# rfrazier716/PyRayT

Hardware: AMD Instinct MI355X
Metric: ray-surface intersections/sec, 1M-ray biconvex lens (higher is better)
Workload: dtype f64

## Files before the change

include/prt.h:

```cpp
#ifndef PRT_H
#define PRT_H

#include <stdint.h>

#ifdef __cplusplus
extern "C" {
#endif

#define PRT_VERSION 240

enum {
  PRT_ROW_OX = 0, PRT_ROW_OY = 1, PRT_ROW_OZ = 2, PRT_ROW_OW = 3,
  PRT_ROW_DX = 4, PRT_ROW_DY = 5, PRT_ROW_DZ = 6, PRT_ROW_DW = 7,
  PRT_ROW_GENERATION = 8, PRT_ROW_INTENSITY = 9, PRT_ROW_WAVELENGTH = 10,
  PRT_ROW_INDEX = 11, PRT_ROW_ID = 12,
  PRT_RAY_ROWS = 13
};

enum {
  PRT_COL_GENERATION = 0, PRT_COL_INTENSITY = 1, PRT_COL_WAVELENGTH = 2, PRT_COL_INDEX = 3,
  PRT_COL_ID = 4, PRT_COL_SURFACE = 5, PRT_COL_X0 = 6, PRT_COL_Y0 = 7, PRT_COL_Z0 = 8,
  PRT_COL_X1 = 9, PRT_COL_Y1 = 10, PRT_COL_Z1 = 11, PRT_COL_XTILT = 12, PRT_COL_YTILT = 13,
  PRT_COL_ZTILT = 14,
  PRT_RECORD_COLS = 15
// ... 52 lines not shown

typedef struct prt_scene_options {
  int32_t struct_size;
  int32_t no_chain;
  int32_t no_cull;
  int32_t cull_min;
  int32_t no_groups;
  int32_t no_implied;
  int32_t hit_lanes;
  int32_t hit_staged;
  int32_t list_order_groups;
  int32_t one_direction;
  int32_t no_intervals;
  int32_t no_clearance;
  int32_t no_plane_bound;
  int32_t reserved[3];
} prt_scene_options;

int prt_scene_create(const prt_prim* prims, int n_prims, const prt_node* nodes, int n_nodes,
                     const int32_t* roots, int n_roots, const prt_material* mats, int n_mats,
                     const prt_scene_options* options, prt_scene** out);
void prt_scene_destroy(prt_scene* scene);
int prt_scene_update(prt_scene* scene, const prt_prim* prims, int n_prims, const prt_node* nodes, int n_nodes,
                     const int32_t* roots, int n_roots, const prt_material* mats, int n_mats,
                     const prt_scene_options* options);
int prt_scene_set_index_tables(prt_scene* scene, const int64_t* ranges, int n_mats, const double* wavelengths,
                               const double* indices, int64_t total);
int prt_scene_component_rows(const prt_scene* scene, int root);
int prt_scene_info(const prt_scene* scene, int64_t* out10);


// ... 216 lines not shown
                                                     int64_t max_group_rows);
int prt_frame_design_sensitivity(int device, const double* rows, int64_t ld, const int64_t* rows_per_generation,
                                 int n_generations, double id0, int64_t n_ids, const prt_prim* surfaces, int n_surfaces,
                                 const double* twists, const int64_t* parameter_ids, const int32_t* parameter_first,
                                 const double* linear, const double* index_rates, const int64_t* index_ids,
                                 const int32_t* index_first, int n_parameters, const int64_t* row_slot,
                                 const int64_t* selected, int64_t n_selected, const int64_t* group_first, int n_groups,
                                 int weight_column, const double* pivots, double* jacobian_out, double* sums_out,
                                 int64_t* record_out, void* workspace, void* stream);

#define PRT_VARIANT_FUSED 1
#define PRT_VARIANT_UNFUSED 2
#define PRT_VARIANT_KLANES 3
int prt_trace_stats(const prt_scene* scene, double* out8);
int prt_trace_telemetry(const prt_scene* scene, int64_t* out12);
int prt_trace_shortcut_counts(const prt_scene* scene, int64_t* out1);

typedef struct prt_camera {
  double world[16];
  int64_t h_pixels, v_pixels;
  double h_width, v_width;
} prt_camera;

int prt_camera_rays(int device, const prt_camera* camera, int64_t first, int64_t count,
                    double* rays_out, int64_t ld, void* stream);

int prt_render_hits(prt_scene* scene, int device, const double* rays, int64_t n, int64_t ld,
                    double* t_out, int64_t* surf_out, void* stream);

int prt_gooch_shade(prt_scene* scene, int device, const double* rays, int64_t n, int64_t ld,
                    const double* t, const int64_t* surf, const double* gooch,
// ... 53 lines not shown
```

pyrayt_amd/csrc/prt_abi_states.hpp:

```cpp
#pragma once
extern "C" int prt_version(void) { return PRT_VERSION; }
extern "C" const char* prt_last_error(void) { return g_error.c_str(); }
extern "C" int prt_device_count(void) {
  int count = 0;
  if (hipGetDeviceCount(&count) != hipSuccess) return 0;
  return count;
}

static inline unsigned blocks_for(int64_t n) { return (unsigned)((n + PRT_BLOCK - 1) / PRT_BLOCK); }
static inline size_t lds_bytes(int slots) { return (size_t)slots * PRT_BLOCK * 12; }
static inline size_t align_up(size_t v, size_t a) { return (v + a - 1) / a * a; }
static inline size_t lds_bytes_fused(int slots) {
  return (size_t)((3 * slots + 1) / 2 + 8) * PRT_BLOCK * sizeof(double);
}

static SceneDev trace_scene_dev(const prt_scene* s, const DeviceCopy* c) {
  SceneDev sd{c->prims, c->trace_code, (int)s->trace_program.code.size(), s->trace_program.lds_slots};
  for (size_t p = 0; p < s->dev_prims.size() && p < 64; ++p)
    if (s->dev_prims[p].mat_kind == MAT_ABSORBER) sd.absorber_mask |= 1ull << p;
  return sd;
}

struct HitVariant {
  int lanes = 1;
// ... 190 lines not shown
  const InteractLayout l = interact_layout(n);
  char* w = (char*)workspace;
  TraceCtrl* ctrl = (TraceCtrl*)(w + l.ctrl);
  int32_t* counts = (int32_t*)(w + l.counts);
  int64_t* offsets = (int64_t*)(w + l.offsets);
  hipLaunchKernelGGL(k_ctrl_init, dim3(1), dim3(1), 0, st, ctrl, n, ld_rows);
  if (n > 0) {
    SceneDev sd{c->prims, nullptr, (int)s->prims.size(), 0};
    hipLaunchKernelGGL(k_count, dim3(blocks_for(n)), dim3(PRT_BLOCK), 0, st, sd,
                       (int)s->prims.size(), rays_in, ld_in, n, surf, counts);
    hipLaunchKernelGGL(k_scan, dim3(1), dim3(1024), 0, st, counts, offsets, ctrl);
    const int relaunch = (generation + 1 != generation_limit) ? 1 : 0;
    hipLaunchKernelGGL(k_shade, dim3(blocks_for(n)), dim3(PRT_BLOCK), 0, st, sd, rays_in, ld_in,
                       (const TraceCtrl*)ctrl, n, t, (const int32_t*)nullptr, surf,
                       (const int64_t*)offsets, rays_out, ld_out, rows_out, ld_rows, (int64_t)0,
                       (double)(generation + 1), relaunch, ray_offset, 1, ctrl, shaded, ld_shaded);
  }
  hipLaunchKernelGGL(k_interact_finish, dim3(1), dim3(1), 0, st, (const TraceCtrl*)ctrl, n_live_out);
  HIP_TRY(hipGetLastError());
  return PRT_OK;
}

#include "prt_host_shade.hpp"
```

pyrayt_amd/csrc/prt_device.hpp:

```cpp
#pragma once
#include <hip/hip_runtime.h>
#include <stdint.h>

#include "prt_math.hpp"

#ifndef PRT_BLOCK
#define PRT_BLOCK 256
#endif
#define PRT_INF (__builtin_inf())

struct DevPrim {
  double minv[16];
  double params[6];
  double coef[6];
  double surface_id;
  int32_t type, mat_kind, normal_scale, pad;
};

typedef const __attribute__((address_space(4))) DevPrim* ConstPrimPtr;
__device__ __forceinline__ ConstPrimPtr const_prim(const DevPrim* prims, int index) {
  return (ConstPrimPtr)(unsigned long long)(prims + index);
}

enum { I_LEAF = 0, I_CSG = 1, I_ROOT = 2, I_BOX = 3, I_CHAIN = 4 };
enum { BOX_TEST = 0, BOX_PICK = 1, BOX_JUMP = 2, BOX_LINE = 3 };
enum { OPER_REGA = 0, OPER_REGB = 1, OPER_LDS = 2 };
enum { CSG_UNION = 1, CSG_INTERSECT = 2, CSG_DIFFERENCE = 3 };
enum { PRIM_SPHERE = 0, PRIM_CYLINDER = 1, PRIM_PLANE = 2, PRIM_CUBE = 3, PRIM_PARABOLOID = 4 };
enum { MAT_NONE = 0, MAT_ABSORBER = 1, MAT_MIRROR = 2, MAT_CONST = 3, MAT_SELLMEIER = 4, MAT_TABLE = 5, MAT_HOST = 6 };

struct DevInstr {
// ... 16 lines not shown
  int32_t shape;
  int32_t n_leaves;
  int32_t op1, op2;
  int32_t prim[3];
  int32_t implied1, implied2;
  int32_t clearance;
  int32_t intervals;
  double box1[6], box2[6];
  double leaf[3][18];
};
static_assert(sizeof(DevChain) == 3 * sizeof(DevInstr), "a chain record spans three step slots");
enum { CHAIN_SLOTS = 3 };
enum {
  CHAIN_SSC = 0, CHAIN_SSQ, CHAIN_CSS, CHAIN_QSS, CHAIN_QQQ,
  CHAIN_SC, CHAIN_SQ, CHAIN_CS, CHAIN_QS, CHAIN_CB, CHAIN_QB, CHAIN_PC, CHAIN_PQ, CHAIN_BC,
  CHAIN_SHAPES
};

struct Ray8 {
  double ox, oy, oz, ow, dx, dy, dz, dw;
  bool gated;
  bool any_w;
  bool lex;
  unsigned long long* paths;
};

#define kWellFormedLen2Lo 0.81
__device__ __forceinline__ bool well_formed(const Ray8& r) {
  if (!r.gated) return false;
  const double len2 = (r.dx * r.dx + r.dy * r.dy) + r.dz * r.dz;
// ... 204 lines not shown
  t0 = fmin(h0, h1);
  t1 = fmax(h0, h1);
}
__device__ __forceinline__ void surface_pair(int type, const double* __restrict__ q,
                                             const double* __restrict__ m, const Ray8& r,
                                             double& t0, double& t1) {
  const double ox = row_dot(m, 0, r.ox, r.oy, r.oz, r.ow);
  const double oy = row_dot(m, 1, r.ox, r.oy, r.oz, r.ow);
  const double oz = row_dot(m, 2, r.ox, r.oy, r.oz, r.ow);
  const double dx = row_dot(m, 0, r.dx, r.dy, r.dz, r.dw);
  const double dy = row_dot(m, 1, r.dx, r.dy, r.dz, r.dw);
  const double dz = row_dot(m, 2, r.dx, r.dy, r.dz, r.dw);
  object_pair(type, q, ox, oy, oz, dx, dy, dz, t0, t1);
}

__device__ __forceinline__ void plane_leaf_candidate(const double* __restrict__ q, const double* __restrict__ m,
                                                     const Ray8& r, int p, double& best_t, int& best_prim) {
  const double oz = row_dot(m, 2, r.ox, r.oy, r.oz, r.ow);
  const double dz = row_dot(m, 2, r.dx, r.dy, r.dz, r.dw);
  const bool skew = near0(dz);
  double t = -oz / (dz + (skew ? 1.0 : 0.0));
  if (skew) t = PRT_INF;
  const bool can = t > 0 && t < PRT_INF && beats(r, t, p, best_t, best_prim);
  if (__ballot(can) == 0ull) {
    count_wave(r.paths, 4);
    return;
  }
  const double ox = row_dot(m, 0, r.ox, r.oy, r.oz, r.ow);
  const double oy = row_dot(m, 1, r.ox, r.oy, r.oz, r.ow);
  const double dx = row_dot(m, 0, r.dx, r.dy, r.dz, r.dw);
// ... 26 lines not shown
    case PRIM_PLANE:
      ax = 0.0; ay = 0.0; az = 1.0;
      normalise = false;
      break;
    case PRIM_CUBE:
      ax = close_to(lx, q[1]) ? 1.0 : (close_to(lx, q[0]) ? -1.0 : 0.0);
      ay = close_to(ly, q[3]) ? 1.0 : (close_to(ly, q[2]) ? -1.0 : 0.0);
      az = close_to(lz, q[5]) ? 1.0 : (close_to(lz, q[4]) ? -1.0 : 0.0);
      break;
    default:
      ax = lx; ay = ly; az = -2 * q[0];
      if (close_to(lz, q[1])) { ax = 0.0; ay = 0.0; az = 1.0; }
      break;
  }
  if (normalise) {
    const double len = norm4(ax, ay, az, 0.0);
    div3(ax, ay, az, len, ax, ay, az);
  }
}

template <class PrimPtr>
__device__ __forceinline__ void world_normal_len(PrimPtr p, double px, double py, double pz, double pw,
                                                 double& nx, double& ny, double& nz, double& len_out) {
  const auto m = p->minv;
  const double lx = row_dot(m, 0, px, py, pz, pw);
  const double ly = row_dot(m, 1, px, py, pz, pw);
  const double lz = row_dot(m, 2, px, py, pz, pw);
  const auto q = p->params;
  double ax, ay, az;
  bool normalise = true;
  switch (p->type) {
// ... 8 lines not shown
    case PRIM_PLANE:
      ax = 0.0; ay = 0.0; az = 1.0;
      normalise = false;
      break;
    case PRIM_CUBE:
      ax = close_to(lx, q[1]) ? 1.0 : (close_to(lx, q[0]) ? -1.0 : 0.0);
      ay = close_to(ly, q[3]) ? 1.0 : (close_to(ly, q[2]) ? -1.0 : 0.0);
      az = close_to(lz, q[5]) ? 1.0 : (close_to(lz, q[4]) ? -1.0 : 0.0);
      break;
    default:
      ax = lx; ay = ly; az = -2 * q[0];
      if (close_to(lz, q[1])) { ax = 0.0; ay = 0.0; az = 1.0; }
      break;
  }
  if (normalise) {
    const double len = norm4(ax, ay, az, 0.0);
    ax /= len; ay /= len; az /= len;
  }
  double wx = col_dot(m, 0, ax, ay, az, 0.0);
  double wy = col_dot(m, 1, ax, ay, az, 0.0);
  double wz = col_dot(m, 2, ax, ay, az, 0.0);
  const double len = norm4(wx, wy, wz, 0.0);
  const double sgn = (double)p->normal_scale;
  div3(wx, wy, wz, len, wx, wy, wz);
  nx = wx * sgn;
  ny = wy * sgn;
  nz = wz * sgn;
  len_out = len;
}
template <class PrimPtr>
__device__ __forceinline__ void world_normal(PrimPtr p, double px, double py, double pz, double pw,
                                             double& nx, double& ny, double& nz) {
  double len;
  world_normal_len(p, px, py, pz, pw, nx, ny, nz, len);
}

template <class PrimPtr>
// ... 23 lines not shown
                  (k[2] * w2) / (w2 - k[5]));
}

__device__ __forceinline__ void reflect4(double& dx, double& dy, double& dz, double& dw, double nx,
                                         double ny, double nz, double nw) {
  const double dot = ((dx * nx + dy * ny) + dz * nz) + dw * nw;
  dx = dx - (2 * nx) * dot;
  dy = dy - (2 * ny) * dot;
  dz = dz - (2 * nz) * dot;
  dw = dw - (2 * nw) * dot;
}

__device__ __forceinline__ void refract4(double vx, double vy, double vz, double vw, double nx,
                                         double ny, double nz, double nw, double n1, double n2_in,
                                         double n_global, double& ox, double& oy, double& oz,
                                         double& ow, double& index_out) {
  const double cos_p = ((vx * nx + vy * ny) + vz * nz) + vw * nw;
  const double cos_n = ((vx * -nx + vy * -ny) + vz * -nz) + vw * -nw;
  const bool leaving = cos_p > 0;
  const double n2 = leaving ? n_global : n2_in;
  const double mx = leaving ? -nx : nx, my = leaving ? -ny : ny, mz = leaving ? -nz : nz,
               mw = leaving ? -nw : nw;
  const double r = n1 / n2;
  const double cos1 = leaving ? cos_p : cos_n;
  const double radicand = 1 - (r * r) * (1 - cos1 * cos1);
  const double cos2 = prt_sqrt_clamped(radicand);
  double ux, uy, uz, uw;
  if (radicand > 0) {
    const double k = r * cos1 - cos2;
    ux = r * vx + k * mx; uy = r * vy + k * my; uz = r * vz + k * mz; uw = r * vw + k * mw;
  } else {
    const double k = 2 * cos1;
    ux = vx + k * mx; uy = vy + k * my; uz = vz + k * mz; uw = vw + k * mw;
  }
  const double ulen = norm4(ux, uy, uz, uw);
  div3(ux, uy, uz, ulen, ox, oy, oz);
  ow = uw;
  if (uw != 0.0 || !(ulen > 0.0 && ulen < PRT_INF)) ow = uw / ulen;
  index_out = (radicand > 0) ? n2 : n1;
}

template <class PrimPtr>
__device__ __forceinline__ int shade(PrimPtr p, double px, double py, double pz, double pw, double& dx,
                                     double& dy, double& dz, double& dw, double wavelength,
                                     double& index, double tx, double ty, double tz) {
  const int kind = p->mat_kind;
  if (kind == MAT_NONE || kind == MAT_HOST) return -5;
  if (kind == MAT_ABSORBER) {
    dx = 0.0; dy = 0.0; dz = 0.0; dw = 0.0;
    return 0;
  }
  double nx, ny, nz;
  world_normal(p, px, py, pz, pw, nx, ny, nz);
  const double nw = 0.0 * (double)p->normal_scale;
  if (kind == MAT_MIRROR) {
    reflect4(dx, dy, dz, dw, nx, ny, nz, nw);
    return 0;
  }
  bool found;
  const double n_mat = glass_index(p, wavelength, found);
  double vx = tx, vy = ty, vz = tz, vw = dw;
  if (dw != 0.0) {
    const double len = norm4(dx, dy, dz, dw);
    vx = dx / len; vy = dy / len; vz = dz / len; vw = dw / len;
  }
  refract4(vx, vy, vz, vw, nx, ny, nz, nw, index, n_mat, 1.0, dx, dy, dz, dw, index);
  return found ? 0 : -6;
}

extern __shared__ double lds_dyn[];

struct LaneLists {
  int total;
  int off;
  __device__ __forceinline__ double get_t(int slot) const {
    return lds_dyn[(off + slot) * PRT_BLOCK + threadIdx.x];
  }
  __device__ __forceinline__ int get_id(int slot) const {
    return reinterpret_cast<const int*>(lds_dyn + total * PRT_BLOCK)[(off + slot) * PRT_BLOCK + threadIdx.x];
  }
  __device__ __forceinline__ void put(int slot, double v, int i) const {
// ... 311 lines not shown
  return inside;
}

__device__ __forceinline__ void offer_chord(const Ray8& ray, bool some, double lo, double hi, int id_lo, int id_hi,
                                            double& best_t, int& best_prim) {
  const bool first = some && lo > 0;
  const bool second = some && hi > 0 && hi < PRT_INF;
  const double t = first ? lo : (second ? hi : PRT_INF);
  const int prim = first ? id_lo : (second ? id_hi : -1);
  if (beats(ray, t, prim, best_t, best_prim)) {
    best_t = t;
    best_prim = prim;
  }
}

template <int T0, int T1, int T2>
__device__ __forceinline__ void chain_candidate(const DevChain* __restrict__ ch, const Ray8& ray,
                                                double& best_t, int& best_prim) {
  double lv[2], rv[2], r2[2] = {PRT_INF, PRT_INF};
  const int id0 = ch->prim[0], id1 = ch->prim[1];
  bool have_third = false;
  if (T0 == PRIM_CYLINDER && T2 >= 0 && ch->intervals != 0 && ch->clearance != 0) {
    surface_pair(T1, ch->leaf[1], ch->leaf[1] + 6, ray, rv[0], rv[1]);
    surface_pair(T2 < 0 ? 0 : T2, ch->leaf[2], ch->leaf[2] + 6, ray, r2[0], r2[1]);
    have_third = true;
    const int id2 = ch->prim[2];
    const bool b_in = r2[0] >= rv[0], b_out = r2[1] < rv[1];
    const double lo = b_in ? r2[0] : rv[0], hi = b_out ? r2[1] : rv[1];
    const bool tie = lo == hi && hi < PRT_INF;
    bool some = lo < hi;
    const bool wanted = (some && hi > 0) || tie;
    if (__ballot(wanted) == 0ull) return;
    if (__ballot(wanted && (tie || !chord_inside_cylinder(ch->leaf[0], ch->leaf[0] + 6, ray, lo, hi))) == 0ull) {
      some = some && implied_touch(ch->box1, ray, some, lo, hi);
      some = some && implied_touch(ch->box2, ray, some, lo, hi);
      offer_chord(ray, some, lo, hi, b_in ? id2 : id1, b_out ? id2 : id1, best_t, best_prim);
      return;
    }
    surface_pair(T0, ch->leaf[0], ch->leaf[0] + 6, ray, lv[0], lv[1]);
  } else {
    surface_pair(T0, ch->leaf[0], ch->leaf[0] + 6, ray, lv[0], lv[1]);
    surface_pair(T1, ch->leaf[1], ch->leaf[1] + 6, ray, rv[0], rv[1]);
  }
  if (ch->intervals != 0) {
    const bool b_in = rv[0] >= lv[0], b_out = rv[1] < lv[1];
    double lo = b_in ? rv[0] : lv[0], hi = b_out ? rv[1] : lv[1];
    int id_lo = b_in ? id1 : id0, id_hi = b_out ? id1 : id0;
    bool undecided = lo == hi && hi < PRT_INF;
    bool some = lo < hi;
    some = some && implied_touch(ch->box1, ray, some, lo, hi);
    if (T2 >= 0) {
      const bool wanted = (some && hi > 0) || undecided;
      if (__ballot(wanted) == 0ull) return;
      bool cut = true;
// ... 44 lines not shown
    csg_keep<4, 2>(op2, l4, r2, ch->box2, ray, implied2, keep4, keep2, c2);
    const int id2 = ch->prim[2];
    const int lid[4] = {id0, id0, id1, id1}, rid[2] = {id2, id2};
    csg_root_pick<4, 2>(l4, lid, keep4, r2, rid, keep2, t, prim);
  }
  if (beats(ray, t, prim, best_t, best_prim)) {
    best_t = t;
    best_prim = prim;
  }
}

__device__ __forceinline__ void chain_step(const DevChain* __restrict__ ch, int shape, const Ray8& ray,
                                           double& best_t, int& best_prim) {
  switch (shape) {
    case CHAIN_SSC: chain_candidate<PRIM_SPHERE, PRIM_SPHERE, PRIM_CYLINDER>(ch, ray, best_t, best_prim); break;
    case CHAIN_SSQ: chain_candidate<PRIM_SPHERE, PRIM_SPHERE, PRIM_CUBE>(ch, ray, best_t, best_prim); break;
    case CHAIN_CSS: chain_candidate<PRIM_CYLINDER, PRIM_SPHERE, PRIM_SPHERE>(ch, ray, best_t, best_prim); break;
    case CHAIN_QSS: chain_candidate<PRIM_CUBE, PRIM_SPHERE, PRIM_SPHERE>(ch, ray, best_t, best_prim); break;
    case CHAIN_QQQ: chain_candidate<PRIM_CUBE, PRIM_CUBE, PRIM_CUBE>(ch, ray, best_t, best_prim); break;
    case CHAIN_SC: chain_candidate<PRIM_SPHERE, PRIM_CYLINDER, -1>(ch, ray, best_t, best_prim); break;
    case CHAIN_SQ: chain_candidate<PRIM_SPHERE, PRIM_CUBE, -1>(ch, ray, best_t, best_prim); break;
    case CHAIN_CS: chain_candidate<PRIM_CYLINDER, PRIM_SPHERE, -1>(ch, ray, best_t, best_prim); break;
    case CHAIN_QS: chain_candidate<PRIM_CUBE, PRIM_SPHERE, -1>(ch, ray, best_t, best_prim); break;
    case CHAIN_CB: chain_candidate<PRIM_CYLINDER, PRIM_PARABOLOID, -1>(ch, ray, best_t, best_prim); break;
    case CHAIN_QB: chain_candidate<PRIM_CUBE, PRIM_PARABOLOID, -1>(ch, ray, best_t, best_prim); break;
    case CHAIN_PC: chain_candidate<PRIM_PLANE, PRIM_CYLINDER, -1>(ch, ray, best_t, best_prim); break;
    case CHAIN_PQ: chain_candidate<PRIM_PLANE, PRIM_CUBE, -1>(ch, ray, best_t, best_prim); break;
    default: chain_candidate<PRIM_PARABOLOID, PRIM_CYLINDER, -1>(ch, ray, best_t, best_prim); break;
  }
}
// ... 175 lines not shown
```

pyrayt_amd/csrc/prt_scene.hpp:

```cpp
#pragma once
static thread_local std::string g_error;

static int fail(int code, const std::string& msg) {
  g_error = msg;
  return code;
}

#define HIP_TRY(expr)                                                                        \
  do {                                                                                       \
    hipError_t e_ = (expr);                                                                  \
    if (e_ != hipSuccess)                                                                    \
      return fail(PRT_ERR_HIP, std::string(#expr) + ": " + hipGetErrorString(e_));          \
  } while (0)

static const int kMaxBatch = 64;
struct SceneDev {
  const DevPrim* prims;
  const DevInstr* code;
  int n_instr;
  int lds_slots;
  unsigned long long absorber_mask = 0;
};

struct Program {
// ... 92 lines not shown
  std::vector<int64_t> table_ranges;
  std::vector<double> table_wavelengths, table_indices;
  bool has_cull_steps = false;
  bool spatial_groups = false;
  int stats_device = -1, stats_ticket = 0;
  int last_generations = 0;
  long lookback_fallbacks = 0;
  int64_t hint_n = -1;
  int hint_keep_absorbed = 0;
  std::vector<char> hint_mode;
  long speculation_misses = 0;
  bool full_rows = false;
  long full_rows_fallbacks = 0;
  long dense_launches = 0;
  long sparse_keep_launches = 0;
  long long path_counts[5] = {0, 0, 0, 0, 0};
  int hint_holdoff = 0;
  std::vector<char> missed_mode;
  std::vector<int> hint_rest, hint_rest_span;
  int hint_misses_in_a_row = 0;
};

static int leaves_under(const prt_scene* s, int node) {
  const prt_node& n = s->nodes[node];
  if (n.op == PRT_NODE_LEAF) return 1;
  return leaves_under(s, n.left) + leaves_under(s, n.right);
}

static bool solid_bounds(const prt_scene* s, int node, double* box);

static double short_direction_bound(const prt_scene* s, int node);
// ... 261 lines not shown
  out->implied1 = c.box_contains_solid(nodes[0]) ? 1 : 0;
  for (int k = 0; k < 6; ++k) out->box1[k] = s->nodes[nodes[0]].aabb[k];
  if (n_leaves == 3) {
    out->op2 = s->nodes[nodes[1]].op;
    out->implied2 = c.box_contains_solid(nodes[1]) ? 1 : 0;
    for (int k = 0; k < 6; ++k) out->box2[k] = s->nodes[nodes[1]].aabb[k];
  }
  for (int k = 0; k < n_leaves; ++k) {
    const int prim = s->nodes[leaves[k]].prim;
    const prt_prim& pr = s->prims[prim];
    out->prim[k] = prim;
    for (int j = 0; j < 6; ++j) out->leaf[k][j] = pr.params[j];
    for (int j = 0; j < 12; ++j) out->leaf[k][6 + j] = pr.minv[j];
  }
  out->clearance = s->options.no_clearance ? 0 : 1;
  out->intervals = (out->op1 == PRT_NODE_INTERSECT && out->implied1 && (n_leaves == 2 || (out->op2 == PRT_NODE_INTERSECT && out->implied2))) ? 1 : 0;
  if (s->options.no_intervals) out->intervals = 0;
  return true;
}
static Operand compile_component(const prt_scene* s, int root_node, std::vector<DevInstr>& code,
                                 int root_rule, int* slots) {
  size_t box_at = (size_t)-1;
  const bool cull_off = s->options.no_cull != 0;
  const int cull_min = s->options.cull_min > 0 ? s->options.cull_min : 3;
  const bool line_cull = root_rule == ROOT_RENDER && !cull_off;
  if ((root_rule == ROOT_TRACE && (int)s->roots.size() >= cull_min && !cull_off) || line_cull) {
    DevInstr in = Compiler::blank(I_BOX);
    in.a1 = line_cull ? BOX_LINE : BOX_TEST;
    double* box = in.data;
    if (solid_bounds(s, root_node, box) && short_direction_bound(s, root_node) <= kWellFormedLen2Lo) {
// ... 365 lines not shown
    }
    const prt_material& m = s->mats[p.material];
    if (m.kind < PRT_MAT_NONE || m.kind > PRT_MAT_HOST) {
      delete s;
      return fail(PRT_ERR_SCENE, "unknown material kind");
    }
    DevPrim d;
    std::memset(&d, 0, sizeof(d));
    std::memcpy(d.minv, p.minv, sizeof(d.minv));
    std::memcpy(d.params, p.params, sizeof(d.params));
    std::memcpy(d.coef, m.coef, sizeof(d.coef));
    d.surface_id = (double)p.surface_id;
    d.type = p.type;
    d.mat_kind = m.kind;
    d.normal_scale = p.normal_scale < 0 ? -1 : 1;
    if (m.kind == PRT_MAT_NONE || m.kind == PRT_MAT_HOST || m.kind == PRT_MAT_TABLE) s->has_untracable = true;
    if (m.kind == PRT_MAT_TABLE) {
      const double nan_index = m.coef[3];
      std::memset(d.coef, 0, sizeof(d.coef));
      d.coef[3] = nan_index;
    }
    s->dev_prims.push_back(d);
  }
  compile_trace_program(s);
  if (const char* wrong = verify_program(s, s->trace_program, true)) {
    const std::string message = std::string("internal error, the compiled trace program is malformed: ") + wrong;
    delete s;
    return fail(PRT_ERR_SCENE, message);
  }
  s->has_cull_steps = count_steps(s->trace_program.code, I_BOX) > 0;
// ... 313 lines not shown
```

pyrayt_amd/csrc/prt_trace_kernels.hpp:

```cpp
#pragma once
__device__ __forceinline__ LaneLists lane_lists(int slots) { return LaneLists{slots, 0}; }

__device__ __forceinline__ Ray8 load_ray8(const double* __restrict__ rays, int64_t ld, int64_t i) {
  Ray8 r;
  r.ox = rays[0 * ld + i]; r.oy = rays[1 * ld + i]; r.oz = rays[2 * ld + i]; r.ow = rays[3 * ld + i];
  r.dx = rays[4 * ld + i]; r.dy = rays[5 * ld + i]; r.dz = rays[6 * ld + i]; r.dw = rays[7 * ld + i];
  r.gated = false;
  r.any_w = true;
  r.lex = false;
  r.paths = nullptr;
  return r;
}

struct TraceCtrl {
  int64_t n_cur;
  int64_t n_live;
  int64_t n_carry;
  int64_t row_base;
  int64_t rows_cap;
  int32_t error;
  int32_t pad;
  unsigned long long paths[6];
};

// ... 185 lines not shown

struct Meta5 {
  double generation, intensity, wavelength, index, id;
};
__device__ __forceinline__ Meta5 load_meta(const double* __restrict__ rays, int64_t ld, int64_t i) {
  Meta5 m;
  m.generation = rays[8 * ld + i];
  m.intensity = rays[9 * ld + i];
  m.wavelength = rays[10 * ld + i];
  m.index = rays[11 * ld + i];
  m.id = rays[12 * ld + i];
  return m;
}

__device__ __forceinline__ Shaded interact_compute(const SceneDev& scene, const Meta5& m, const Ray8& r,
                                                   double t, int prim) {
  Shaded s;
  s.generation = m.generation;
  s.intensity = m.intensity;
  s.wavelength = m.wavelength;
  s.index_in = m.index;
  s.id = m.id;
  s.px = r.ox + r.dx * t; s.py = r.oy + r.dy * t; s.pz = r.oz + r.dz * t; s.pw = r.ow + r.dw * t;
  s.dx = r.dx; s.dy = r.dy; s.dz = r.dz; s.dw = r.dw;
  s.index = s.index_in;
  s.surface_id = -1.0;
  s.err = 0;
  const double tilt = norm3(r.dx, r.dy, r.dz);
  div3(r.dx, r.dy, r.dz, tilt, s.tx, s.ty, s.tz);
  unsigned long long todo = __ballot(true);
  while (todo) {
    const int leader = __ffsll((long long)todo) - 1;
    const int cur = __shfl(prim, leader);
    if (prim == cur) {
      const DevPrim* __restrict__ p = scene.prims + cur;
      s.err = shade(p, s.px, s.py, s.pz, s.pw, s.dx, s.dy, s.dz, s.dw, s.wavelength, s.index,
                   s.tx, s.ty, s.tz);
      s.surface_id = p->surface_id;
    }
    todo &= ~__ballot(prim == cur);
  }
  return s;
}

__device__ __forceinline__ void interact_store(const Shaded& s, const Ray8& r, bool carry, int64_t row,
                                               int64_t j, double* __restrict__ next, int64_t ld_next,
                                               double* __restrict__ rows, int64_t ld_rows,
                                               double next_generation, int relaunch, double ray_offset) {
  rows[PRT_COL_GENERATION * ld_rows + row] = s.generation;
  rows[PRT_COL_INTENSITY * ld_rows + row] = s.intensity;
  rows[PRT_COL_WAVELENGTH * ld_rows + row] = s.wavelength;
  rows[PRT_COL_INDEX * ld_rows + row] = s.index_in;
// ... 35 lines not shown
                                              bool carry, int64_t row, int64_t j,
                                              double* __restrict__ next, int64_t ld_next,
                                              double* __restrict__ rows, int64_t ld_rows,
                                              double next_generation, int relaunch, double ray_offset) {
  const Shaded s = interact_compute(scene, load_meta(rays, ld, i), r, t, prim);
  interact_store(s, r, carry, row, j, next, ld_next, rows, ld_rows, next_generation, relaunch, ray_offset);
  return s.err;
}

__global__ void __launch_bounds__(PRT_BLOCK)
k_shade(SceneDev scene, const double* __restrict__ rays, int64_t ld, const TraceCtrl* __restrict__ ctrl_in,
        int64_t n_fixed, const double* __restrict__ hit_t, const int32_t* __restrict__ hit_prim,
        const int64_t* __restrict__ hit_surf, const int64_t* __restrict__ block_offsets,
        double* __restrict__ next, int64_t ld_next, double* __restrict__ rows, int64_t ld_rows,
        int64_t row_base_fixed, double next_generation, int relaunch, double ray_offset,
        int keep_absorbed, TraceCtrl* __restrict__ ctrl, const double* __restrict__ shaded, int64_t ld_shaded) {
  __shared__ int s_wave[4];
  const int64_t n = ctrl_in ? ctrl_in->n_cur : n_fixed;
  if (ctrl_in && (ctrl_in->error != 0 || ctrl_in->n_live == 0)) return;
  const int64_t row_base = ctrl_in ? ctrl_in->row_base : row_base_fixed;
  const int64_t i = (int64_t)blockIdx.x * PRT_BLOCK + threadIdx.x;
  const bool in_range = i < n;
  Ray8 r = {0, 0, 0, 1, 0, 0, 0, 0};
  double t = PRT_INF;
  int prim = -1;
  if (in_range) {
    r = load_ray8(rays, ld, i);
    t = hit_t[i];
    if (hit_prim) {
      prim = hit_prim[i];
    } else {
      prim = prim_of_surface(scene.prims, scene.n_instr, hit_surf[i]);
    }
  }
  const bool live = in_range && is_live(r, prim);
  const bool carry = live && (keep_absorbed || scene.prims[prim].mat_kind != MAT_ABSORBER);
  const int live_rank = block_rank(live, s_wave);
  const int carry_rank = block_rank(carry, s_wave);
  if (!live) return;

  const int64_t row = row_base + block_offsets[2 * blockIdx.x] + live_rank;
  const int64_t j = block_offsets[2 * blockIdx.x + 1] + carry_rank;
// ... 551 lines not shown
                 (last >> 6);
        finisher = done;
      }
    }
  } else if (threadIdx.x == 0 && tile > 0) {
    tile_store(tiles_cur + tile, tile_pack(TILE_AGGREGATE, agg_live, agg_carry));
  }
  Shaded sh;
  sh.err = 0;
  STAMP(4);
  if (live) {
    Meta5 meta = {0, 0, 0, 0, 0};
    meta.wavelength = PARK(2);
    meta.index = PARK(3);
    PARK(5) = r.ox; PARK(6) = r.oy; PARK(7) = r.oz;
    sh = interact_compute(scene, meta, r, t, prim);
  }
  STAMP(5);
  const int64_t last_tile = (n - 1) / PRT_BLOCK;
  int64_t excl_live, excl_carry;
  if (!PLAN && assume >= 5) {
    __syncthreads();
    excl_live = s_excl[0];
    excl_carry = s_excl[1];
  } else if (assume) {
    excl_live = rec_none ? 0 : (int64_t)tile * PRT_BLOCK;
    excl_carry = carry_form == 1 ? (int64_t)tile * PRT_BLOCK : 0;
  } else {
  if (wave == 0) {
    unsigned e_live, e_carry;
    bool ok = lookback(tiles_cur, tile, agg_live, agg_carry, e_live, e_carry, &ctrl->error);
// ... 193 lines not shown
```

pyrayt_amd/csrc/prt_trace_runtime.hpp:

```cpp
#pragma once
struct TraceLayout {
  size_t ctrl, fctrl, gen, dead_lists, gen_rows, tiles_a, tiles_b, counts, offsets, hit_t, hit_prim, rays_a,
      rays_b, total;
};
static TraceLayout trace_layout(int64_t n) {
  const size_t nb = blocks_for(n) + 1;
  const size_t nn = (size_t)(n < 1 ? 1 : n);
  TraceLayout l;
  size_t at = 0;
  auto take = [&](size_t bytes) { size_t here = at; at += align_up(bytes, 256); return here; };
  l.ctrl = take(sizeof(TraceCtrl));
  l.fctrl = take(sizeof(GenCtrl) + (kMaxGenerationSlots + 1) * sizeof(GenCtrl));
  l.gen = l.fctrl + sizeof(GenCtrl);
  l.dead_lists = take(3 * sizeof(DeadList));
  l.gen_rows = take(kMaxGenerationSlots * sizeof(int64_t));
  l.tiles_a = take(nb * sizeof(unsigned long long));
  l.tiles_b = take(nb * sizeof(unsigned long long));
  l.counts = take(nb * 2 * sizeof(int32_t));
  l.offsets = take(nb * 2 * sizeof(int64_t));
  l.hit_t = take(nn * sizeof(double));
  l.hit_prim = take(nn * sizeof(int32_t));
  l.rays_a = take(nn * PRT_RAY_ROWS * sizeof(double));
  l.rays_b = take(nn * PRT_RAY_ROWS * sizeof(double));
  l.total = at;
// ... 58 lines not shown
  for (int g = 0; g < generation_limit && n_cur > 0; ++g) {
    double* dst = buf[g & 1];
    const unsigned nb = blocks_for(n_cur);
    const int relaunch = (g + 1 != generation_limit) ? 1 : 0;
    HIP_TRY(hipEventRecord(t->ev0, st));
    {
      int rc_hit = launch_hit(s, c, sd, st, src, src_ld, (const TraceCtrl*)ctrl, (int64_t)0, n_cur, hit_t, hit_prim,
                              (int64_t*)nullptr, counts, keep_absorbed, count_paths ? ctrl->paths : nullptr);
      if (rc_hit) return rc_hit;
    }
    hipLaunchKernelGGL(k_scan, dim3(1), dim3(1024), 0, st, (const int32_t*)counts, offsets, ctrl);
    hipLaunchKernelGGL(k_shade, dim3(nb), dim3(PRT_BLOCK), 0, st, sd, src, src_ld,
                       (const TraceCtrl*)ctrl, (int64_t)0, (const double*)hit_t,
                       (const int32_t*)hit_prim, (const int64_t*)nullptr, (const int64_t*)offsets,
                       dst, n, t->rows_out, t->rows_cap, (int64_t)0, (double)(g + 1), relaunch,
                       t->ray_offset, keep_absorbed, ctrl, (const double*)nullptr, (int64_t)0);
    hipLaunchKernelGGL(k_advance, dim3(1), dim3(1), 0, st, ctrl, gen_rows, g);
    HIP_TRY(hipEventRecord(t->ev1, st));
    static_assert(sizeof(TraceCtrl) <= 12 * sizeof(int64_t), "the control block ends in front of the row count's slot");
    HIP_TRY(hipMemcpyAsync(t->host_pinned, ctrl, sizeof(TraceCtrl), hipMemcpyDeviceToHost, st));
    HIP_TRY(hipMemcpyAsync(t->host_pinned + 12, gen_rows + g, sizeof(int64_t), hipMemcpyDeviceToHost, st));
    HIP_TRY(hipStreamSynchronize(st));
    float ms = 0;
    HIP_TRY(hipEventElapsedTime(&ms, t->ev0, t->ev1));
    const TraceCtrl* h = (const TraceCtrl*)t->host_pinned;
    t->stats[0] += 1;
    t->stats[1] += (double)n_cur;
    t->stats[2] += ms;
    t->stats[3] += 4;
    if (h->error) { error = h->error; break; }
    const int64_t live = t->host_pinned[12];
    rows_per_generation[g] = live;
    total_rows += live;
    t->stats[4] += (double)live;
    t->stats[5] += (double)h->n_cur;
    n_cur = h->n_cur;
    src = dst;
    src_ld = n;
  }
  if (error) return trace_error(error);
  if (count_paths) {
    const TraceCtrl* h = (const TraceCtrl*)t->host_pinned;
    s->path_counts[0] += 1;
    for (int k = 1; k < 5; ++k) s->path_counts[k] += (long long)h->paths[k];
  }
  return total_rows;
}

static const int kGenerationBatch = 4;

static int settle_timing(TraceTicket* t) {
  if (!t->timing_pending) return PRT_OK;
  t->timing_pending = false;
  HIP_TRY(hipEventSynchronize(t->ev1));
  float ms = 0;
  HIP_TRY(hipEventElapsedTime(&ms, t->ev0, t->ev1));
  t->stats[2] += ms;
  return PRT_OK;
}
// ... 646 lines not shown
extern "C" int prt_trace_telemetry(const prt_scene* s, int64_t* out12) {
  int64_t* out8 = out12;
  if (!s || !out8) return fail(PRT_ERR_ARG, "null argument");
  out12[8] = s->plan_launches;
  out12[9] = s->plan_misses;
  out12[10] = s->sparse_keep_launches;
  out12[11] = s->plan_dense_launches;
  out8[0] = s->lookback_fallbacks;
  out8[1] = s->speculation_misses;
  out8[2] = s->dense_launches;
  out8[3] = s->full_rows_fallbacks;
  for (int k = 0; k < 4; ++k) out8[4 + k] = s->path_counts[k];
  return PRT_OK;
}

extern "C" int prt_trace_shortcut_counts(const prt_scene* s, int64_t* out1) {
  if (!s || !out1) return fail(PRT_ERR_ARG, "null argument");
  out1[0] = s->path_counts[4];
  return PRT_OK;
}

extern "C" int prt_trace_stats(const prt_scene* s, double* out8) {
  if (!s || !out8) return fail(PRT_ERR_ARG, "null argument");
  for (int k = 0; k < 8; ++k) out8[k] = 0;
  if (s->stats_device < 0 || s->stats_device >= (int)s->per_device.size()) return PRT_OK;
  TraceTicket* t = &const_cast<prt_scene*>(s)->per_device[s->stats_device].ticket[s->stats_ticket];
  if (!t->active) {
    HIP_TRY(hipSetDevice(s->stats_device));
    int rc = settle_timing(t);
    if (rc) return rc;
  }
  for (int k = 0; k < 8; ++k) out8[k] = t->stats[k];
  return PRT_OK;
// ... 10 lines not shown
```

pyrayt_amd/engine.py:

```python
import ctypes
import os
import warnings
import weakref

import numpy as np

from . import scene as _scene

_HERE = os.path.dirname(os.path.abspath(__file__))
LIB_PATH = os.environ.get("PRT_LIB", os.path.join(_HERE, "csrc", "libprt_hip.so"))


from . import _runtime
from ._runtime import HW_QUEUES

RAY_ROWS = 13
RECORD_COLS = 15
DEFAULT_RAY_OFFSET = 1e-6

TRACE_KEEP_ABSORBED = 1
TRACE_UNFUSED = 2
TRACE_NO_HINTS = 4
TRACE_FULL_ROWS = 8
TRACE_PUBLISH_KERNEL = 16
TRACE_TEST_STALL = 32
TRACE_SYNC = 64
TRACE_COUNT_PATHS = 128
TRACE_NO_TIMING = 256
TRACE_NO_SPARSE_KEEP = 1024
TRACE_BUSY = 2048
TRACE_TICKETS = 4

OPTIONS_DTYPE = np.dtype(
    [("struct_size", "<i4"), ("no_chain", "<i4"), ("no_cull", "<i4"), ("cull_min", "<i4"), ("no_groups", "<i4"),
     ("no_implied", "<i4"), ("hit_lanes", "<i4"), ("hit_staged", "<i4"), ("list_order_groups", "<i4"),
     ("one_direction", "<i4"), ("no_intervals", "<i4"), ("no_clearance", "<i4"), ("no_plane_bound", "<i4"),
     ("reserved", "<i4", (3,))])
assert OPTIONS_DTYPE.itemsize == 64
OPTION_NAMES = tuple(name for name in OPTIONS_DTYPE.names if name not in ("struct_size", "reserved"))
DEFAULT_OPTIONS = {}
DEFAULT_TRACE_FLAGS = 0


def options_record(options=None):
    merged = dict(DEFAULT_OPTIONS)
    merged.update(options or {})
    rec = np.zeros(1, dtype=OPTIONS_DTYPE)
    rec["struct_size"] = OPTIONS_DTYPE.itemsize
    for key, value in merged.items():
        if key not in OPTION_NAMES:
            raise ValueError(f"unknown scene option {key!r} (known: {', '.join(OPTION_NAMES)})")
        rec[key] = int(value)
# ... 651 lines not shown
    def trace_stats(self):
        out = (ctypes.c_double * 8)()
        _check(library().prt_trace_stats(self.handle, out))
        return {"generations": int(out[0]), "ray_generations": int(out[1]),
                "kernel_ms": float(out[2]), "kernel_launches": int(out[3]),
                "rows": int(out[4]), "rays_carried": int(out[5]),
                "lookback_fallbacks": int(out[6]), "variant": int(out[7])}

    def telemetry(self):
        out = (ctypes.c_int64 * 12)()
        _check(library().prt_trace_telemetry(self.handle, out))
        keys = ("lookback_fallbacks", "speculation_misses", "dense_launches", "full_rows_fallbacks",
                "counted_traces", "rays_not_well_formed", "implied_box_nodes", "exact_box_tests",
                "plan_launches", "plan_misses", "sparse_keep_launches", "plan_dense_launches")
        told = dict(zip(keys, (int(v) for v in out)))
        more = (ctypes.c_int64 * 1)()
        _check(library().prt_trace_shortcut_counts(self.handle, more))
        told["plane_leaves_not_finished"] = int(more[0])
        return told

    def propagate(self, rays):
        torch = _torch()
        n = rays.shape[1]
        t = torch.empty(n, dtype=torch.float64, device=rays.device)
        surf = torch.empty(n, dtype=torch.int64, device=rays.device)
        if n:
            _check(library().prt_propagate(self.handle, rays.device.index or 0, rays.data_ptr(), n,
                                           rays.stride(0), t.data_ptr(), surf.data_ptr(),
                                           _stream_ptr(torch, rays.device)))
        return t, surf

    def interact(self, rays, t, surf, generation, generation_limit, ray_offset=DEFAULT_RAY_OFFSET, shaded=None,
                 rows_out=None):
# ... 503 lines not shown
```

Measured before the change: 22.39 billion.

## Share transform partials across chain leaves and take wave-uniform refraction side

When all leaves of a CSG chain share the same 3x3 inverse-transform rows, the ray is partially transformed once and each leaf only adds its own translation column. For two spheres the quadratic 'a' term is reused as well. Refraction uses a wave ballot so a wave whose rays all enter, or all leave, skips the per-lane side selection. The norm4 calls with a zero w are replaced by norm3. This adds new chain shapes and counters, and the ballot adds cross-lane work to every shade call.

```diff
diff --git a/include/prt.h b/include/prt.h
--- a/include/prt.h
+++ b/include/prt.h
@@ -90,7 +90,9 @@
   int32_t no_intervals;
   int32_t no_clearance;
   int32_t no_plane_bound;
-  int32_t reserved[3];
+  int32_t no_shared_transform;
+  int32_t no_wave_sides;
+  int32_t reserved[1];
 } prt_scene_options;
 
 int prt_scene_create(const prt_prim* prims, int n_prims, const prt_node* nodes, int n_nodes,
@@ -337,7 +339,7 @@
 #define PRT_VARIANT_KLANES 3
 int prt_trace_stats(const prt_scene* scene, double* out8);
 int prt_trace_telemetry(const prt_scene* scene, int64_t* out12);
-int prt_trace_shortcut_counts(const prt_scene* scene, int64_t* out1);
+int prt_trace_shortcut_counts(const prt_scene* scene, int64_t* out3);
 
 typedef struct prt_camera {
   double world[16];
diff --git a/pyrayt_amd/csrc/prt_abi_states.hpp b/pyrayt_amd/csrc/prt_abi_states.hpp
--- a/pyrayt_amd/csrc/prt_abi_states.hpp
+++ b/pyrayt_amd/csrc/prt_abi_states.hpp
@@ -228,7 +228,8 @@
     hipLaunchKernelGGL(k_shade, dim3(blocks_for(n)), dim3(PRT_BLOCK), 0, st, sd, rays_in, ld_in,
                        (const TraceCtrl*)ctrl, n, t, (const int32_t*)nullptr, surf,
                        (const int64_t*)offsets, rays_out, ld_out, rows_out, ld_rows, (int64_t)0,
-                       (double)(generation + 1), relaunch, ray_offset, 1, ctrl, shaded, ld_shaded);
+                       (double)(generation + 1), relaunch, ray_offset, 1, ctrl, shaded, ld_shaded,
+                       (unsigned long long*)nullptr);
   }
   hipLaunchKernelGGL(k_interact_finish, dim3(1), dim3(1), 0, st, (const TraceCtrl*)ctrl, n_live_out);
   HIP_TRY(hipGetLastError());
diff --git a/pyrayt_amd/csrc/prt_device.hpp b/pyrayt_amd/csrc/prt_device.hpp
--- a/pyrayt_amd/csrc/prt_device.hpp
+++ b/pyrayt_amd/csrc/prt_device.hpp
@@ -14,7 +14,8 @@
   double params[6];
   double coef[6];
   double surface_id;
-  int32_t type, mat_kind, normal_scale, pad;
+  int32_t type, mat_kind, normal_scale;
+  int32_t wave_sides;
 };
 
 typedef const __attribute__((address_space(4))) DevPrim* ConstPrimPtr;
@@ -61,6 +62,7 @@
 enum {
   CHAIN_SSC = 0, CHAIN_SSQ, CHAIN_CSS, CHAIN_QSS, CHAIN_QQQ,
   CHAIN_SC, CHAIN_SQ, CHAIN_CS, CHAIN_QS, CHAIN_CB, CHAIN_QB, CHAIN_PC, CHAIN_PQ, CHAIN_BC,
+  CHAIN_SSC_ONE, CHAIN_CSS_ONE, CHAIN_SC_ONE, CHAIN_CS_ONE,
   CHAIN_SHAPES
 };
 
@@ -295,6 +297,57 @@
   object_pair(type, q, ox, oy, oz, dx, dy, dz, t0, t1);
 }
 
+struct RowPartials {
+  double ox, oy, oz, dx, dy, dz;
+};
+__device__ __forceinline__ double row_partial(const double* __restrict__ m, int r, double x, double y, double z) {
+  double acc = m[4 * r + 0] * x;
+  acc = fma(m[4 * r + 1], y, acc);
+  acc = fma(m[4 * r + 2], z, acc);
+  return acc;
+}
+__device__ __forceinline__ RowPartials row_partials(const double* __restrict__ m, const Ray8& r) {
+  RowPartials p;
+  p.ox = row_partial(m, 0, r.ox, r.oy, r.oz); p.oy = row_partial(m, 1, r.ox, r.oy, r.oz);
+  p.oz = row_partial(m, 2, r.ox, r.oy, r.oz);
+  p.dx = row_partial(m, 0, r.dx, r.dy, r.dz); p.dy = row_partial(m, 1, r.dx, r.dy, r.dz);
+  p.dz = row_partial(m, 2, r.dx, r.dy, r.dz);
+  return p;
+}
+__device__ __forceinline__ void finish_rows(const double* __restrict__ m, const Ray8& r, const RowPartials& p, double& ox,
+                                            double& oy, double& oz, double& dx, double& dy, double& dz) {
+  ox = fma(m[3], r.ow, p.ox); oy = fma(m[7], r.ow, p.oy); oz = fma(m[11], r.ow, p.oz);
+  dx = fma(m[3], r.dw, p.dx); dy = fma(m[7], r.dw, p.dy); dz = fma(m[11], r.dw, p.dz);
+}
+__device__ __forceinline__ void sphere_pair_with_a(const double* __restrict__ q, double ox, double oy, double oz,
+                                                   double dx, double dy, double dz, double a, double& t0, double& t1) {
+  const double b = 2 * ((dx * ox + dy * oy) + dz * oz);
+  const double c = ((ox * ox + oy * oy) + oz * oz) - q[0] * q[0];
+  const double disc = b * b - 4 * a * c;
+  const double s = prt_sqrt_clamped(disc);
+  const double den = 2 * a;
+  double h0, h1;
+  div2(-b + s, -b - s, den, h0, h1);
+  if (!(disc >= 0)) { h0 = PRT_INF; h1 = PRT_INF; }
+  h0 = nan_to_inf(h0);
+  h1 = nan_to_inf(h1);
+  t0 = fmin(h0, h1);
+  t1 = fmax(h0, h1);
+}
+template <int TYPE>
+__device__ __forceinline__ void surface_pair_from(const double* __restrict__ q, const double* __restrict__ m,
+                                                  const Ray8& r, const RowPartials& p, bool take_a, double& a_io,
+                                                  double& t0, double& t1) {
+  double ox, oy, oz, dx, dy, dz;
+  finish_rows(m, r, p, ox, oy, oz, dx, dy, dz);
+  if (TYPE == PRIM_SPHERE) {
+    if (!take_a) a_io = (dx * dx + dy * dy) + dz * dz;
+    sphere_pair_with_a(q, ox, oy, oz, dx, dy, dz, a_io, t0, t1);
+  } else {
+    object_pair(TYPE, q, ox, oy, oz, dx, dy, dz, t0, t1);
+  }
+}
+
 __device__ __forceinline__ void plane_leaf_candidate(const double* __restrict__ q, const double* __restrict__ m,
                                                      const Ray8& r, int p, double& best_t, int& best_prim) {
   const double oz = row_dot(m, 2, r.ox, r.oy, r.oz, r.ow);
@@ -351,7 +404,7 @@
       break;
   }
   if (normalise) {
-    const double len = norm4(ax, ay, az, 0.0);
+    const double len = norm3(ax, ay, az);
     div3(ax, ay, az, len, ax, ay, az);
   }
 }
@@ -390,13 +443,13 @@
       break;
   }
   if (normalise) {
-    const double len = norm4(ax, ay, az, 0.0);
+    const double len = norm3(ax, ay, az);
     ax /= len; ay /= len; az /= len;
   }
   double wx = col_dot(m, 0, ax, ay, az, 0.0);
   double wy = col_dot(m, 1, ax, ay, az, 0.0);
   double wz = col_dot(m, 2, ax, ay, az, 0.0);
-  const double len = norm4(wx, wy, wz, 0.0);
+  const double len = norm3(wx, wy, wz);
   const double sgn = (double)p->normal_scale;
   div3(wx, wy, wz, len, wx, wy, wz);
   nx = wx * sgn;
@@ -450,15 +503,31 @@
 __device__ __forceinline__ void refract4(double vx, double vy, double vz, double vw, double nx,
                                          double ny, double nz, double nw, double n1, double n2_in,
                                          double n_global, double& ox, double& oy, double& oz,
-                                         double& ow, double& index_out) {
-  const double cos_p = ((vx * nx + vy * ny) + vz * nz) + vw * nw;
+                                         double& ow, double& index_out, bool wave_sides = false,
+                                         bool* one_sided = nullptr) {
   const double cos_n = ((vx * -nx + vy * -ny) + vz * -nz) + vw * -nw;
-  const bool leaving = cos_p > 0;
-  const double n2 = leaving ? n_global : n2_in;
-  const double mx = leaving ? -nx : nx, my = leaving ? -ny : ny, mz = leaving ? -nz : nz,
-               mw = leaving ? -nw : nw;
-  const double r = n1 / n2;
-  const double cos1 = leaving ? cos_p : cos_n;
+  double n2, mx, my, mz, mw, r, cos1;
+  const unsigned long long lanes = __ballot(true), out_lanes = __ballot(cos_n < 0);
+  const bool all_in = wave_sides && out_lanes == 0ull, all_out = wave_sides && out_lanes == lanes;
+  if (one_sided != nullptr) *one_sided = all_in || all_out;
+  if (all_in) {
+    n2 = n2_in;
+    mx = nx; my = ny; mz = nz; mw = nw;
+    r = n1 / n2;
+    cos1 = cos_n;
+  } else if (all_out) {
+    n2 = n_global;
+    mx = -nx; my = -ny; mz = -nz; mw = -nw;
+    r = n_global == 1.0 ? n1 : n1 / n2;
+    cos1 = ((vx * nx + vy * ny) + vz * nz) + vw * nw;
+  } else {
+    const double cos_p = ((vx * nx + vy * ny) + vz * nz) + vw * nw;
+    const bool leaving = cos_p > 0;
+    n2 = leaving ? n_global : n2_in;
+    mx = leaving ? -nx : nx; my = leaving ? -ny : ny; mz = leaving ? -nz : nz; mw = leaving ? -nw : nw;
+    r = n1 / n2;
+    cos1 = leaving ? cos_p : cos_n;
+  }
   const double radicand = 1 - (r * r) * (1 - cos1 * cos1);
   const double cos2 = prt_sqrt_clamped(radicand);
   double ux, uy, uz, uw;
@@ -479,7 +548,8 @@
 template <class PrimPtr>
 __device__ __forceinline__ int shade(PrimPtr p, double px, double py, double pz, double pw, double& dx,
                                      double& dy, double& dz, double& dw, double wavelength,
-                                     double& index, double tx, double ty, double tz) {
+                                     double& index, double tx, double ty, double tz,
+                                     unsigned long long* paths = nullptr, bool sides = true) {
   const int kind = p->mat_kind;
   if (kind == MAT_NONE || kind == MAT_HOST) return -5;
   if (kind == MAT_ABSORBER) {
@@ -500,7 +570,10 @@
     const double len = norm4(dx, dy, dz, dw);
     vx = dx / len; vy = dy / len; vz = dz / len; vw = dw / len;
   }
-  refract4(vx, vy, vz, vw, nx, ny, nz, nw, index, n_mat, 1.0, dx, dy, dz, dw, index);
+  bool one_sided = false;
+  refract4(vx, vy, vz, vw, nx, ny, nz, nw, index, n_mat, 1.0, dx, dy, dz, dw, index, sides && p->wave_sides != 0,
+           paths != nullptr ? &one_sided : nullptr);
+  if (paths != nullptr && one_sided) count_wave(paths, 0);
   return found ? 0 : -6;
 }
 
@@ -842,15 +915,25 @@
   }
 }
 
-template <int T0, int T1, int T2>
+template <int T0, int T1, int T2, bool ONE = false>
 __device__ __forceinline__ void chain_candidate(const DevChain* __restrict__ ch, const Ray8& ray,
                                                 double& best_t, int& best_prim) {
   double lv[2], rv[2], r2[2] = {PRT_INF, PRT_INF};
   const int id0 = ch->prim[0], id1 = ch->prim[1];
   bool have_third = false;
+  RowPartials part;
+  double a = 0.0;
   if (T0 == PRIM_CYLINDER && T2 >= 0 && ch->intervals != 0 && ch->clearance != 0) {
-    surface_pair(T1, ch->leaf[1], ch->leaf[1] + 6, ray, rv[0], rv[1]);
-    surface_pair(T2 < 0 ? 0 : T2, ch->leaf[2], ch->leaf[2] + 6, ray, r2[0], r2[1]);
+    if (ONE) {
+      part = row_partials(ch->leaf[1] + 6, ray);
+      surface_pair_from<T1>(ch->leaf[1], ch->leaf[1] + 6, ray, part, false, a, rv[0], rv[1]);
+      surface_pair_from<(T2 < 0 ? 0 : T2)>(ch->leaf[2], ch->leaf[2] + 6, ray, part,
+                                           !ray.any_w && T1 == PRIM_SPHERE && T2 == PRIM_SPHERE, a, r2[0], r2[1]);
+      count_wave(ray.paths, 5);
+    } else {
+      surface_pair(T1, ch->leaf[1], ch->leaf[1] + 6, ray, rv[0], rv[1]);
+      surface_pair(T2 < 0 ? 0 : T2, ch->leaf[2], ch->leaf[2] + 6, ray, r2[0], r2[1]);
+    }
     have_third = true;
     const int id2 = ch->prim[2];
     const bool b_in = r2[0] >= rv[0], b_out = r2[1] < rv[1];
@@ -866,6 +949,12 @@
       return;
     }
     surface_pair(T0, ch->leaf[0], ch->leaf[0] + 6, ray, lv[0], lv[1]);
+  } else if (ONE) {
+    part = row_partials(ch->leaf[0] + 6, ray);
+    surface_pair_from<T0>(ch->leaf[0], ch->leaf[0] + 6, ray, part, false, a, lv[0], lv[1]);
+    surface_pair_from<T1>(ch->leaf[1], ch->leaf[1] + 6, ray, part, !ray.any_w && T0 == PRIM_SPHERE && T1 == PRIM_SPHERE, a,
+                          rv[0], rv[1]);
+    count_wave(ray.paths, 5);
   } else {
     surface_pair(T0, ch->leaf[0], ch->leaf[0] + 6, ray, lv[0], lv[1]);
     surface_pair(T1, ch->leaf[1], ch->leaf[1] + 6, ray, rv[0], rv[1]);
@@ -940,6 +1029,10 @@
                                            double& best_t, int& best_prim) {
   switch (shape) {
     case CHAIN_SSC: chain_candidate<PRIM_SPHERE, PRIM_SPHERE, PRIM_CYLINDER>(ch, ray, best_t, best_prim); break;
+    case CHAIN_SSC_ONE: chain_candidate<PRIM_SPHERE, PRIM_SPHERE, PRIM_CYLINDER, true>(ch, ray, best_t, best_prim); break;
+    case CHAIN_CSS_ONE: chain_candidate<PRIM_CYLINDER, PRIM_SPHERE, PRIM_SPHERE, true>(ch, ray, best_t, best_prim); break;
+    case CHAIN_SC_ONE: chain_candidate<PRIM_SPHERE, PRIM_CYLINDER, -1, true>(ch, ray, best_t, best_prim); break;
+    case CHAIN_CS_ONE: chain_candidate<PRIM_CYLINDER, PRIM_SPHERE, -1, true>(ch, ray, best_t, best_prim); break;
     case CHAIN_SSQ: chain_candidate<PRIM_SPHERE, PRIM_SPHERE, PRIM_CUBE>(ch, ray, best_t, best_prim); break;
     case CHAIN_CSS: chain_candidate<PRIM_CYLINDER, PRIM_SPHERE, PRIM_SPHERE>(ch, ray, best_t, best_prim); break;
     case CHAIN_QSS: chain_candidate<PRIM_CUBE, PRIM_SPHERE, PRIM_SPHERE>(ch, ray, best_t, best_prim); break;
diff --git a/pyrayt_amd/csrc/prt_scene.hpp b/pyrayt_amd/csrc/prt_scene.hpp
--- a/pyrayt_amd/csrc/prt_scene.hpp
+++ b/pyrayt_amd/csrc/prt_scene.hpp
@@ -130,7 +130,7 @@
   long full_rows_fallbacks = 0;
   long dense_launches = 0;
   long sparse_keep_launches = 0;
-  long long path_counts[5] = {0, 0, 0, 0, 0};
+  long long path_counts[7] = {0, 0, 0, 0, 0, 0, 0};
   int hint_holdoff = 0;
   std::vector<char> missed_mode;
   std::vector<int> hint_rest, hint_rest_span;
@@ -422,6 +422,21 @@
     for (int j = 0; j < 12; ++j) out->leaf[k][6 + j] = pr.minv[j];
   }
   out->clearance = s->options.no_clearance ? 0 : 1;
+  if (!s->options.no_shared_transform) {
+    const double* m0 = s->prims[out->prim[0]].minv;
+    bool one = true;
+    for (int k = 0; k < n_leaves; ++k) {
+      const double* mk = s->prims[out->prim[k]].minv;
+      for (int r = 0; r < 3; ++r) {
+        one = one && std::memcmp(m0 + 4 * r, mk + 4 * r, 3 * sizeof(double)) == 0;
+        for (int j = 0; j < 4; ++j) one = one && std::isfinite(mk[4 * r + j]);
+      }
+    }
+    static const int one_shape[][2] = {{CHAIN_SSC, CHAIN_SSC_ONE}, {CHAIN_CSS, CHAIN_CSS_ONE}, {CHAIN_SC, CHAIN_SC_ONE},
+                                       {CHAIN_CS, CHAIN_CS_ONE}};
+    for (const auto& pair : one_shape)
+      if (one && out->shape == pair[0]) out->shape = pair[1];
+  }
   out->intervals = (out->op1 == PRT_NODE_INTERSECT && out->implied1 && (n_leaves == 2 || (out->op2 == PRT_NODE_INTERSECT && out->implied2))) ? 1 : 0;
   if (s->options.no_intervals) out->intervals = 0;
   return true;
@@ -817,6 +832,7 @@
     d.type = p.type;
     d.mat_kind = m.kind;
     d.normal_scale = p.normal_scale < 0 ? -1 : 1;
+    d.wave_sides = (s->options.no_wave_sides & 1) ? 0 : 1;
     if (m.kind == PRT_MAT_NONE || m.kind == PRT_MAT_HOST || m.kind == PRT_MAT_TABLE) s->has_untracable = true;
     if (m.kind == PRT_MAT_TABLE) {
       const double nan_index = m.coef[3];
diff --git a/pyrayt_amd/csrc/prt_trace_kernels.hpp b/pyrayt_amd/csrc/prt_trace_kernels.hpp
--- a/pyrayt_amd/csrc/prt_trace_kernels.hpp
+++ b/pyrayt_amd/csrc/prt_trace_kernels.hpp
@@ -223,7 +223,7 @@
 }
 
 __device__ __forceinline__ Shaded interact_compute(const SceneDev& scene, const Meta5& m, const Ray8& r,
-                                                   double t, int prim) {
+                                                   double t, int prim, bool sides = true) {
   Shaded s;
   s.generation = m.generation;
   s.intensity = m.intensity;
@@ -244,7 +244,7 @@
     if (prim == cur) {
       const DevPrim* __restrict__ p = scene.prims + cur;
       s.err = shade(p, s.px, s.py, s.pz, s.pw, s.dx, s.dy, s.dz, s.dw, s.wavelength, s.index,
-                   s.tx, s.ty, s.tz);
+                   s.tx, s.ty, s.tz, r.paths, sides);
       s.surface_id = p->surface_id;
     }
     todo &= ~__ballot(prim == cur);
@@ -310,7 +310,8 @@
         const int64_t* __restrict__ hit_surf, const int64_t* __restrict__ block_offsets,
         double* __restrict__ next, int64_t ld_next, double* __restrict__ rows, int64_t ld_rows,
         int64_t row_base_fixed, double next_generation, int relaunch, double ray_offset,
-        int keep_absorbed, TraceCtrl* __restrict__ ctrl, const double* __restrict__ shaded, int64_t ld_shaded) {
+        int keep_absorbed, TraceCtrl* __restrict__ ctrl, const double* __restrict__ shaded, int64_t ld_shaded,
+        unsigned long long* __restrict__ paths) {
   __shared__ int s_wave[4];
   const int64_t n = ctrl_in ? ctrl_in->n_cur : n_fixed;
   if (ctrl_in && (ctrl_in->error != 0 || ctrl_in->n_live == 0)) return;
@@ -322,6 +323,7 @@
   int prim = -1;
   if (in_range) {
     r = load_ray8(rays, ld, i);
+    r.paths = paths;
     t = hit_t[i];
     if (hit_prim) {
       prim = hit_prim[i];
@@ -903,7 +905,7 @@
     meta.wavelength = PARK(2);
     meta.index = PARK(3);
     PARK(5) = r.ox; PARK(6) = r.oy; PARK(7) = r.oz;
-    sh = interact_compute(scene, meta, r, t, prim);
+    sh = interact_compute(scene, meta, r, t, prim, !PLAN);
   }
   STAMP(5);
   const int64_t last_tile = (n - 1) / PRT_BLOCK;
diff --git a/pyrayt_amd/csrc/prt_trace_runtime.hpp b/pyrayt_amd/csrc/prt_trace_runtime.hpp
--- a/pyrayt_amd/csrc/prt_trace_runtime.hpp
+++ b/pyrayt_amd/csrc/prt_trace_runtime.hpp
@@ -96,7 +96,8 @@
                        (const TraceCtrl*)ctrl, (int64_t)0, (const double*)hit_t,
                        (const int32_t*)hit_prim, (const int64_t*)nullptr, (const int64_t*)offsets,
                        dst, n, t->rows_out, t->rows_cap, (int64_t)0, (double)(g + 1), relaunch,
-                       t->ray_offset, keep_absorbed, ctrl, (const double*)nullptr, (int64_t)0);
+                       t->ray_offset, keep_absorbed, ctrl, (const double*)nullptr, (int64_t)0,
+                       count_paths ? ctrl->paths : (unsigned long long*)nullptr);
     hipLaunchKernelGGL(k_advance, dim3(1), dim3(1), 0, st, ctrl, gen_rows, g);
     HIP_TRY(hipEventRecord(t->ev1, st));
     static_assert(sizeof(TraceCtrl) <= 12 * sizeof(int64_t), "the control block ends in front of the row count's slot");
@@ -124,7 +125,8 @@
   if (count_paths) {
     const TraceCtrl* h = (const TraceCtrl*)t->host_pinned;
     s->path_counts[0] += 1;
-    for (int k = 1; k < 5; ++k) s->path_counts[k] += (long long)h->paths[k];
+    for (int k = 1; k < 6; ++k) s->path_counts[k] += (long long)h->paths[k];
+    s->path_counts[6] += (long long)h->paths[0];
   }
   return total_rows;
 }
@@ -801,9 +803,9 @@
   return PRT_OK;
 }
 
-extern "C" int prt_trace_shortcut_counts(const prt_scene* s, int64_t* out1) {
-  if (!s || !out1) return fail(PRT_ERR_ARG, "null argument");
-  out1[0] = s->path_counts[4];
+extern "C" int prt_trace_shortcut_counts(const prt_scene* s, int64_t* out3) {
+  if (!s || !out3) return fail(PRT_ERR_ARG, "null argument");
+  for (int k = 0; k < 3; ++k) out3[k] = s->path_counts[4 + k];
   return PRT_OK;
 }
 
diff --git a/pyrayt_amd/engine.py b/pyrayt_amd/engine.py
--- a/pyrayt_amd/engine.py
+++ b/pyrayt_amd/engine.py
@@ -35,7 +35,7 @@
     [("struct_size", "<i4"), ("no_chain", "<i4"), ("no_cull", "<i4"), ("cull_min", "<i4"), ("no_groups", "<i4"),
      ("no_implied", "<i4"), ("hit_lanes", "<i4"), ("hit_staged", "<i4"), ("list_order_groups", "<i4"),
      ("one_direction", "<i4"), ("no_intervals", "<i4"), ("no_clearance", "<i4"), ("no_plane_bound", "<i4"),
-     ("reserved", "<i4", (3,))])
+     ("no_shared_transform", "<i4"), ("no_wave_sides", "<i4"), ("reserved", "<i4", (1,))])
 assert OPTIONS_DTYPE.itemsize == 64
 OPTION_NAMES = tuple(name for name in OPTIONS_DTYPE.names if name not in ("struct_size", "reserved"))
 DEFAULT_OPTIONS = {}
@@ -717,9 +717,9 @@
                 "counted_traces", "rays_not_well_formed", "implied_box_nodes", "exact_box_tests",
                 "plan_launches", "plan_misses", "sparse_keep_launches", "plan_dense_launches")
         told = dict(zip(keys, (int(v) for v in out)))
-        more = (ctypes.c_int64 * 1)()
+        more = (ctypes.c_int64 * 3)()
         _check(library().prt_trace_shortcut_counts(self.handle, more))
-        told["plane_leaves_not_finished"] = int(more[0])
+        told["plane_leaves_not_finished"], told["chains_sharing_a_transform"], told["one_sided_turns"] = (int(v) for v in more)
         return told
 
     def propagate(self, rays):
```

Result: slower. 21.94 billion (-2.0%).
